# struan-robertson/shoeprint-image-retrieval

Hardware: AMD Instinct MI355X
Metric: query x gallery NCC pairs/sec (higher is better)
Workload: dtype f32; 1 GPU; config 2: WVU2019-shaped VGG16 conv3_3 NCC: Q=100 x G=1500 (1500/GPU), features [256,128,64] stored as float32, rotations/scales none, queries signal 1 / noise 126; method=fft, gallery_chunk=1500, storage=float32, parallelism=gallery-shard x1, streams=1

## Files before the change

### shoeprint-image-retrieval_amd/csrc/ncc_prep6.hip

```cpp
#include "fft_core.h"
#include "ncc_fft_cfg.h"
#include "ncc_prep_common.h"

namespace spr {
namespace {

using C6 = Cfg<12, 16, 12, 8, 384, 5, 2, 1>;
constexpr int kPT = 512;
constexpr int kLoads = 16;
constexpr int kSeg = 4;
constexpr int kRowSeg = 16;
constexpr int kChansPerWg = 8;

#ifdef SPR_PREP6_STAMPS
__device__ unsigned long long g_prep6_stamps[16];
#define SPR_PSTAMP6(i) do { if (blockIdx.x == 12 && blockIdx.y == 700 && c == c_first + 1 && threadIdx.x == 0) g_prep6_stamps[i] = __builtin_amdgcn_s_memtime(); } while (0)
#else
#define SPR_PSTAMP6(i)
#endif

struct Prep6Lds {
  size_t x0_off, f_off, xbuf_off, tw_off, total;
  int f_stride;
};
Prep6Lds prep6_lds(const NccGeom& g) {
  const int h = g.ih, w = g.iw;
  Prep6Lds l;
  l.f_stride = C6::NW / 2 + 1;
  const size_t f_bytes = sizeof(cf) * static_cast<size_t>(2 * ((h + 1) / 2)) * l.f_stride;
  l.x0_off = 64;
  l.f_off = align_up(l.x0_off + sizeof(float) * h * w, 16);
  l.xbuf_off = align_up(l.f_off + f_bytes, 16);
  const size_t fft_total = l.xbuf_off + sizeof(cf) * C6::prep_xbuf_elems(kPT);
  const size_t stat_total = l.f_off + 2 * sizeof(double) * static_cast<size_t>(h) * w;
  l.tw_off = align_up(fft_total > stat_total ? fft_total : stat_total, 16);
  l.total = l.tw_off + sizeof(cf) * (C6::NW + C6::NH);
  return l;
}

__device__ __forceinline__ void stretch_offsets(double t, int sg, int d, double& off, double& tot) {
  const double a = shfl_xor(t, d), b = shfl_xor(t, 2 * d), c = shfl_xor(t, 3 * d);
  off = 0.0;
  tot = 0.0;
#pragma unroll
  for (int j = 0; j < kSeg; ++j) {
    const double v = j == sg ? t : (j == (sg ^ 1) ? a : (j == (sg ^ 2) ? b : c));
    off += j < sg ? v : 0.0;
    tot += v;
  }
}

__global__ void __launch_bounds__(kPT)
prep6_gallery_kernel(NccGeom g, const void* __restrict__ maps, unsigned char* __restrict__ prepared, size_t item_bytes,
                     const cf* __restrict__ tw_h, const cf* __restrict__ tw_w, unsigned x0_off, unsigned f_off,
                     unsigned xbuf_off, unsigned tw_off, int f_stride) {
  using C = C6;
  using GH = typename C::GH;
  using GW = typename C::GW;
  unsigned char* lds = dyn_lds();
  double* red = reinterpret_cast<double*>(lds);
  float* x0 = reinterpret_cast<float*>(lds + x0_off);
  cf* F = reinterpret_cast<cf*>(lds + f_off);
  cf* xbuf = reinterpret_cast<cf*>(lds + xbuf_off);
  const int tid = static_cast<int>(threadIdx.x);
  const size_t item = blockIdx.y;
  const int h = g.ih, w = g.iw, n = h * w;
  double* H1 = reinterpret_cast<double*>(lds + f_off);
  double* H2 = H1 + n;
  const int c_first = static_cast<int>(blockIdx.x) * kChansPerWg;
  const int c_end = c_first + kChansPerWg < g.channels ? c_first + kChansPerWg : g.channels;

  unsigned char* item_base = prepared + item * item_bytes;
  const size_t spec_bytes = sizeof(cf) * static_cast<size_t>(g.channels) * C::kSpecPerChan;
  unsigned char* flags = item_base + spec_bytes + sizeof(float) * static_cast<size_t>(g.channels) * g.inv_per_chan;

  const int dy = kPT / w, dx = kPT - dy * w;
  const int y_first = tid / w, x_first = tid - y_first * w;
  float v[kLoads];
  auto request = [&](int c) {
    const size_t chan_base = (item * g.channels + c) * static_cast<size_t>(g.g_h) * g.g_w;
    int yy = y_first, xx = x_first;
#pragma unroll
    for (int k = 0; k < kLoads; ++k) {
      v[k] = tid + k * kPT < n
                 ? load_feature(maps, chan_base + static_cast<size_t>(yy + g.crop) * g.g_w + (xx + g.crop), g.dtype)
                 : 0.0f;
      xx += dx; yy += dy;
      if (xx >= w) { xx -= w; ++yy; }
    }
  };
  request(c_first);

  cf* twt_w = reinterpret_cast<cf*>(lds + tw_off);
  cf* twt_h = twt_w + C::NW;
  for (int k = tid; k < C::NW; k += kPT) twt_w[k] = tw_w[(k / C::TGW) * (k % C::TGW)];
  for (int k = tid; k < C::NH; k += kPT) twt_h[k] = tw_h[(k / C::TGH) * (k % C::TGH)];

  const int cy = g.th / 2, cx = g.tw / 2;
  const int above = g.th - cy, left = g.tw - cx;
  const double inv_n = 1.0 / (static_cast<double>(g.th) * static_cast<double>(g.tw));

  for (int c = c_first; c < c_end; ++c) {
    SPR_PSTAMP6(0);
    double s = 0.0;
#pragma unroll
    for (int k = 0; k < kLoads; ++k)
      if (tid + k * kPT < n) s += static_cast<double>(v[k]);
    const double total = block_sum(s, red);
    const float mean = static_cast<float>(total / static_cast<double>(n));
    double e = 0.0;
#pragma unroll
    for (int k = 0; k < kLoads; ++k) {
      if (tid + k * kPT < n) {
        const float d = v[k] - mean;
        x0[tid + k * kPT] = d;
        const float sq = d * d;
        e += static_cast<double>(sq);
      }
    }
    SPR_PSTAMP6(1);
    const float energy = static_cast<float>(block_sum(e, red));
    const float rs = energy > 0.0f ? static_cast<float>(1.0 / sqrt(static_cast<double>(energy))) : 0.0f;
    if (tid == 0) flags[c] = rs == 0.0f ? 1 : 0;
    if (c + 1 < c_end) request(c + 1);
    SPR_PSTAMP6(2);

    {
      const int tidv = opaque(tid);
      const int u = tidv < h * kSeg ? tidv : h * kSeg - 1;
      const bool live = tidv < h * kSeg;
      const int y = u / kSeg, sg = u - y * kSeg;
      const int wseg = (w + kSeg - 1) / kSeg;
      const int xa = sg * wseg < w ? sg * wseg : w;
      const int cnt = w - xa < wseg ? w - xa : wseg;
      const float* src = x0 + y * w;
      float tv[kRowSeg];
#pragma unroll
      for (int k = 0; k < kRowSeg; ++k) {
        const float t = src[xa + k < w ? xa + k : w - 1];
        tv[k] = k < cnt ? t : 0.0f;
      }
      double r1 = 0.0, r2 = 0.0;
#pragma unroll
      for (int k = 0; k < kRowSeg; ++k) {
        const float sq = tv[k] * tv[k];
        r1 += static_cast<double>(tv[k]);
        r2 += static_cast<double>(sq);
      }
      double q1, q2, t1, t2;
      stretch_offsets(r1, sg, 1, q1, t1);
      stretch_offsets(r2, sg, 1, q2, t2);
      double* h1 = H1 + y * w;
      double* h2 = H2 + y * w;
      if (live) {
#pragma unroll
        for (int k = 0; k < kRowSeg; ++k) {
          const float sq = tv[k] * tv[k];
          q1 += static_cast<double>(tv[k]);
          q2 += static_cast<double>(sq);
          const int kk = xa + k + 1;
          if (k < cnt && kk < w) {
            const int xl = kk - left;
            if (xl >= 0 && xl <= cx) { h1[xl] = q1; h2[xl] = q2; }
            const int xr = kk + cx;
            if (xr < w) { h1[xr] = t1 - q1; h2[xr] = t2 - q2; }
          }
        }
        if (cnt > 0 && xa + cnt == w) {
          int xl = w - left < 0 ? 0 : w - left;
          const int xe = cx < w - 1 ? cx : w - 1;
          for (; xl <= xe; ++xl) { h1[xl] = q1; h2[xl] = q2; }
        }
      }
    }
    __syncthreads();
    SPR_PSTAMP6(7);

    {
      const int tidv = opaque(tid);
      const int xcol = ((tidv >> 6) & 3) * 16 + (tidv & 15), csg = (tidv >> 4) & 3;
      const int hseg = (h + kSeg - 1) / kSeg;
      const int ya = csg * hseg < h ? csg * hseg : h;
      const int ycnt = xcol < w ? (h - ya < hseg ? h - ya : hseg) : 0;
      double* col = ((tidv >> 8) ? H2 : H1) + ya * w + (xcol < w ? xcol : w - 1);
      constexpr int B = 8;
      double r = 0.0;
      for (int k0 = 0; k0 < ycnt; k0 += B) {
        double t[B];
#pragma unroll
        for (int k = 0; k < B; ++k) t[k] = col[(k0 + k < ycnt ? k0 + k : ycnt - 1) * w];
#pragma unroll
        for (int k = 0; k < B; ++k) r += k0 + k < ycnt ? t[k] : 0.0;
      }
      double run, tot;
      stretch_offsets(r, csg, 16, run, tot);
      for (int k0 = 0; k0 < ycnt; k0 += B) {
        double t[B];
#pragma unroll
        for (int k = 0; k < B; ++k) t[k] = col[(k0 + k < ycnt ? k0 + k : ycnt - 1) * w];
#pragma unroll
        for (int k = 0; k < B; ++k) {
          run += k0 + k < ycnt ? t[k] : 0.0;
          col[(k0 + k < ycnt ? k0 + k : ycnt - 1) * w] = run;
        }
      }
    }
    __syncthreads();
    SPR_PSTAMP6(8);
    {
      float4* inv4 = reinterpret_cast<float4*>(item_base + spec_bytes) + static_cast<size_t>(c) * (g.inv_per_chan / 4);
      for (int idx4 = opaque(tid); idx4 < C::kInv6PerChan / 4; idx4 += kPT) {
        const int pp = idx4 / C::NT, lane6 = idx4 - pp * C::NT;
        const int l64 = lane6 & 63, rg = l64 / 3, tq = l64 - 3 * rg;
        const int row = (lane6 >> 6) * C::kRowGroups + rg, n1 = 3 * pp + tq;
        float o[4] = {0.0f, 0.0f, 0.0f, 0.0f};
        if (l64 < 63 && n1 < 16 && row < h) {
          const int b = (33 * n1) % 48;
          const int ma = tq == 1 ? b - 32 : b, mb = ma == n1 ? n1 + 16 : n1;
          const bool upper = row <= cy;
          const int hi = upper ? (row + above < h ? row + above : h) - 1 : h - 1;
          const int lo = upper ? 0 : row - cy - 1;
          const double* p1a = H1 + hi * w;
          const double* p1b = H1 + lo * w;
          const double* p2a = H2 + hi * w;
          const double* p2b = H2 + lo * w;
          double a1[4], b1[4], a2[4], b2[4];
#pragma unroll
          for (int e = 0; e < 4; ++e) {
            const int x = 2 * (e < 2 ? ma : mb) + (e & 1), xs = x < w ? x : w - 1;
            a1[e] = p1a[xs]; b1[e] = p1b[xs]; a2[e] = p2a[xs]; b2[e] = p2b[xs];
          }
#pragma unroll
          for (int e = 0; e < 4; ++e) {
            const int x = 2 * (e < 2 ? ma : mb) + (e & 1);
            const float r = inv_sigma_from_sums(upper ? a1[e] : a1[e] - b1[e], upper ? a2[e] : a2[e] - b2[e], inv_n);
            o[e] = x < w ? r : 0.0f;
          }
        }
        inv4[idx4] = float4{o[0], o[1], o[2], o[3]};
      }
    }
    __syncthreads();
    SPR_PSTAMP6(3);

    {
      const int tidv = opaque(tid);
      const int giw = tidv / C::TGW, t = tidv - giw * C::TGW;
      const LdsTwiddles<C::TGW> twr{twt_w, t};
      cf* gbuf = xbuf + giw * C::kRowGroupElems;
      cf* zb = gbuf;
      const int pairs = (h + 1) / 2;
      constexpr int kPairsPerRound = kPT / C::TGW;
      const int rounds = ceil_div(pairs, kPairsPerRound);
      for (int rr = 0; rr < rounds; ++rr) {
        const int pr = rr * kPairsPerRound + giw;
        const int ra = 2 * pr, rb = ra + 1;
        cf x[C::EW], y[GW::SPL][C::TGW];
#pragma unroll
        for (int m = 0; m < C::EW; ++m) {
          const int n2 = GW::in_index(t, m);
          const bool in = n2 < w;
          x[m].x = (in && ra < h) ? x0[ra * w + n2] : 0.0f;
          x[m].y = (in && rb < h) ? x0[rb * w + n2] : 0.0f;
        }
        group_fft<C::EW, C::TGW, -1>(x, y, t, twr, gbuf);
        wave_sync();
#pragma unroll
        for (int pp = 0; pp < GW::SPL; ++pp)
#pragma unroll
          for (int sidx = 0; sidx < C::TGW; ++sidx)
            if (GW::out_valid(t, pp)) zb[GW::out_index(t, pp, sidx)] = y[pp][sidx];
        wave_sync();
        if (pr < pairs) {
          for (int k = t; k <= C::NW / 2; k += C::TGW) {
            const cf zk = zb[k];
            const cf zm = zb[k == 0 ? 0 : C::NW - k];
            F[ra * f_stride + k] = cmake(0.5f * (zk.x + zm.x), 0.5f * (zk.y - zm.y));
            F[rb * f_stride + k] = cmake(0.5f * (zk.y + zm.y), 0.5f * (zm.x - zk.x));
          }
        }
        wave_sync();
      }
    }
    __syncthreads();
    SPR_PSTAMP6(4);

    {
      cf* spec = reinterpret_cast<cf*>(item_base) + static_cast<size_t>(c) * C::kSpecPerChan;
      const int tidv = opaque(tid);
      const int gi = tidv / C::TGH, t = tidv - gi * C::TGH;
      const LdsTwiddles<C::TGH> twc{twt_h, t};
      cf* gbuf = xbuf + gi * GH::kGroupElems;
      const int rows_f = 2 * ((h + 1) / 2);
      constexpr int kColsPerRound = kPT / C::TGH;
      constexpr int kRounds = (C::COLS + 1 + kColsPerRound - 1) / kColsPerRound;
      for (int rc = 0; rc < kRounds; ++rc) {
        const int j = rc * kColsPerRound + gi;
        const bool nyq = j == C::COLS;
        const bool active = j <= C::COLS;
        cf x[C::EH], y[GH::SPL][C::TGH];
#pragma unroll
        for (int m = 0; m < C::EH; ++m) {
          const int n1 = GH::in_index(t, m);
          x[m] = (active && n1 < rows_f) ? F[n1 * f_stride + j] : cmake(0.0f, 0.0f);
        }
        group_fft<C::EH, C::TGH, -1>(x, y, t, twc, gbuf);
        if (active) {
#pragma unroll
          for (int pp = 0; pp < GH::SPL; ++pp) {
            if (!GH::out_valid(t, pp)) continue;
#pragma unroll
            for (int sidx = 0; sidx < C::TGH; ++sidx) {
              const int k1 = GH::out_index(t, pp, sidx);
              spec[nyq ? C::kNyqOffset + k1 : C::spec_index(C::slot(j), k1)] = y[pp][sidx];
            }
          }
        }
      }
    }
    __syncthreads();
    SPR_PSTAMP6(5);
  }
}

}

bool prep6_covers(const NccGeom& g) {
  if (!g.six || g.big || !g.prep6) return false;
  if (g.nh != C6::NH || g.nw != C6::NW || g.nt != C6::NT) return false;
  if (g.th < g.ih || g.tw < g.iw) return false;
  if (g.ih > C6::kRows6 || g.ih * kSeg > kPT || g.iw > 64) return false;
  if (g.ih * g.iw > kLoads * kPT) return false;
  if (g.inv_per_chan != C6::kInv6PerChan) return false;
  return prep6_lds(g).total <= static_cast<size_t>(kLdsLimit);
}

int launch_prep6(const NccGeom& g, const PlanScratch& s, const PrepCall& c) {
  const Prep6Lds l = prep6_lds(g);
  const size_t item_bytes = prepared_gallery_item_bytes(g, SPR_NCC_FFT);
  (void)hipFuncSetAttribute(reinterpret_cast<const void*>(prep6_gallery_kernel),
                            hipFuncAttributeMaxDynamicSharedMemorySize, kLdsLimit);
  const size_t elem = g.dtype == SPR_F32 ? 4 : 2;
  const size_t raw_item_bytes = static_cast<size_t>(g.channels) * g.g_h * g.g_w * elem;
  const int64_t batch = 65535;
  for (int64_t first = 0; first < c.n; first += batch) {
    const int64_t m = c.n - first < batch ? c.n - first : batch;
    hipLaunchKernelGGL(prep6_gallery_kernel, dim3(ceil_div(g.channels, kChansPerWg), static_cast<unsigned>(m)), dim3(kPT),
                       l.total, c.stream, g,
                       static_cast<const void*>(static_cast<const unsigned char*>(c.maps) + first * raw_item_bytes),
                       static_cast<unsigned char*>(c.prepared) + first * item_bytes, item_bytes, s.tw_h, s.tw_w,
                       static_cast<unsigned>(l.x0_off), static_cast<unsigned>(l.f_off), static_cast<unsigned>(l.xbuf_off),
                       static_cast<unsigned>(l.tw_off), l.f_stride);
    const int rc = check_launch("prep6_gallery_kernel");
    if (rc != SPR_OK) return rc;
  }
  return SPR_OK;
}

#ifdef SPR_PREP6_STAMPS
extern "C" int spr_debug_read_prep_stamps(unsigned long long* host, int n) {
  return hipMemcpyFromSymbol(host, HIP_SYMBOL(g_prep6_stamps), sizeof(unsigned long long) * n) == hipSuccess ? 0 : -1;
}
#endif

}
```

Baseline: 279,200 pairs/s.

## Remove energy block reduction and prefetch next-channel sum into reduction slots

The per-channel energy block reduction is replaced with two LDS OR-flags that only check whether any squared deviation is positive or overflow-prone. The exact double energy sum now runs only in that rare overflow case. The next channel's sum is reduced per wave during an existing barrier interval, which removes a block_sum from the critical path. The column prefix scan now holds its whole segment in 32 registers instead of loading twice in chunks of 8, and the row-stretch stores are merged into one branch. These changes cut barriers and LDS traffic at the cost of higher register pressure and an extra syncthreads for the flags.

```diff
diff --git a/shoeprint-image-retrieval_amd/csrc/ncc_prep6.hip b/shoeprint-image-retrieval_amd/csrc/ncc_prep6.hip
--- a/shoeprint-image-retrieval_amd/csrc/ncc_prep6.hip
+++ b/shoeprint-image-retrieval_amd/csrc/ncc_prep6.hip
@@ -10,7 +10,10 @@
 constexpr int kLoads = 16;
 constexpr int kSeg = 4;
 constexpr int kRowSeg = 16;
+constexpr int kColSeg = 32;
 constexpr int kChansPerWg = 8;
+static_assert(kColSeg * kSeg >= C6::kRows6, "a column stretch fits its registers");
+constexpr float kSquareBound = 0x1p100f;
 
 #ifdef SPR_PREP6_STAMPS
 __device__ unsigned long long g_prep6_stamps[16];
@@ -28,7 +31,7 @@
   Prep6Lds l;
   l.f_stride = C6::NW / 2 + 1;
   const size_t f_bytes = sizeof(cf) * static_cast<size_t>(2 * ((h + 1) / 2)) * l.f_stride;
-  l.x0_off = 64;
+  l.x0_off = 80;
   l.f_off = align_up(l.x0_off + sizeof(float) * h * w, 16);
   l.xbuf_off = align_up(l.f_off + f_bytes, 16);
   const size_t fft_total = l.xbuf_off + sizeof(cf) * C6::prep_xbuf_elems(kPT);
@@ -59,6 +62,7 @@
   using GW = typename C::GW;
   unsigned char* lds = dyn_lds();
   double* red = reinterpret_cast<double*>(lds);
+  int* orw = reinterpret_cast<int*>(lds + 64);
   float* x0 = reinterpret_cast<float*>(lds + x0_off);
   cf* F = reinterpret_cast<cf*>(lds + f_off);
   cf* xbuf = reinterpret_cast<cf*>(lds + xbuf_off);
@@ -90,11 +94,19 @@
     }
   };
   request(c_first);
+  auto lane_sum = [&]() {
+    double s = 0.0;
+#pragma unroll
+    for (int k = 0; k < kLoads; ++k)
+      if (tid + k * kPT < n) s += static_cast<double>(v[k]);
+    return s;
+  };
 
   cf* twt_w = reinterpret_cast<cf*>(lds + tw_off);
   cf* twt_h = twt_w + C::NW;
   for (int k = tid; k < C::NW; k += kPT) twt_w[k] = tw_w[(k / C::TGW) * (k % C::TGW)];
   for (int k = tid; k < C::NH; k += kPT) twt_h[k] = tw_h[(k / C::TGH) * (k % C::TGH)];
+  if (tid < 2) orw[tid] = 0;
 
   const int cy = g.th / 2, cx = g.tw / 2;
   const int above = g.th - cy, left = g.tw - cx;
@@ -102,26 +114,45 @@
 
   for (int c = c_first; c < c_end; ++c) {
     SPR_PSTAMP6(0);
-    double s = 0.0;
-#pragma unroll
-    for (int k = 0; k < kLoads; ++k)
-      if (tid + k * kPT < n) s += static_cast<double>(v[k]);
-    const double total = block_sum(s, red);
+    double total = 0.0;
+    if (c == c_first) {
+      total = block_sum(lane_sum(), red);
+    } else {
+#pragma unroll
+      for (int wv = 0; wv < kPT / 64; ++wv) total += red[wv];
+    }
     const float mean = static_cast<float>(total / static_cast<double>(n));
-    double e = 0.0;
+    bool pos = false, big = false;
 #pragma unroll
     for (int k = 0; k < kLoads; ++k) {
       if (tid + k * kPT < n) {
         const float d = v[k] - mean;
         x0[tid + k * kPT] = d;
         const float sq = d * d;
-        e += static_cast<double>(sq);
-      }
-    }
+        pos |= sq > 0.0f;
+        big |= !(sq < kSquareBound);
+      }
+    }
+    if (pos) orw[0] = 1;
+    if (big) orw[1] = 1;
     SPR_PSTAMP6(1);
-    const float energy = static_cast<float>(block_sum(e, red));
-    const float rs = energy > 0.0f ? static_cast<float>(1.0 / sqrt(static_cast<double>(energy))) : 0.0f;
-    if (tid == 0) flags[c] = rs == 0.0f ? 1 : 0;
+    __syncthreads();
+    bool dead = orw[0] == 0;
+    if (orw[1] != 0) {
+      double e = 0.0;
+#pragma unroll
+      for (int k = 0; k < kLoads; ++k) {
+        if (tid + k * kPT < n) {
+          const float d = v[k] - mean;
+          const float sq = d * d;
+          e += static_cast<double>(sq);
+        }
+      }
+      const float energy = static_cast<float>(block_sum(e, red));
+      const float rs = energy > 0.0f ? static_cast<float>(1.0 / sqrt(static_cast<double>(energy))) : 0.0f;
+      dead = rs == 0.0f;
+    }
+    if (tid == 0) flags[c] = dead ? 1 : 0;
     if (c + 1 < c_end) request(c + 1);
     SPR_PSTAMP6(2);
 
@@ -159,11 +190,11 @@
           q1 += static_cast<double>(tv[k]);
           q2 += static_cast<double>(sq);
           const int kk = xa + k + 1;
-          if (k < cnt && kk < w) {
-            const int xl = kk - left;
-            if (xl >= 0 && xl <= cx) { h1[xl] = q1; h2[xl] = q2; }
-            const int xr = kk + cx;
-            if (xr < w) { h1[xr] = t1 - q1; h2[xr] = t2 - q2; }
+          const bool pre = kk >= left;
+          const int xp = pre ? kk - left : kk + cx;
+          if (k < cnt && kk < w && xp <= (pre ? cx : w - 1)) {
+            h1[xp] = pre ? q1 : t1 - q1;
+            h2[xp] = pre ? q2 : t2 - q2;
           }
         }
         if (cnt > 0 && xa + cnt == w) {
@@ -174,6 +205,7 @@
       }
     }
     __syncthreads();
+    if (tid < 2) orw[tid] = 0;
     SPR_PSTAMP6(7);
 
     {
@@ -182,26 +214,21 @@
       const int hseg = (h + kSeg - 1) / kSeg;
       const int ya = csg * hseg < h ? csg * hseg : h;
       const int ycnt = xcol < w ? (h - ya < hseg ? h - ya : hseg) : 0;
-      double* col = ((tidv >> 8) ? H2 : H1) + ya * w + (xcol < w ? xcol : w - 1);
-      constexpr int B = 8;
+      double* col = ((tidv >> 8) ? H2 : H1) + (ycnt > 0 ? ya * w + xcol : 0);
+      const int last = ycnt > 0 ? ycnt - 1 : 0;
+      double t[kColSeg];
+#pragma unroll
+      for (int k = 0; k < kColSeg; ++k) t[k] = col[(k < last ? k : last) * w];
       double r = 0.0;
-      for (int k0 = 0; k0 < ycnt; k0 += B) {
-        double t[B];
-#pragma unroll
-        for (int k = 0; k < B; ++k) t[k] = col[(k0 + k < ycnt ? k0 + k : ycnt - 1) * w];
-#pragma unroll
-        for (int k = 0; k < B; ++k) r += k0 + k < ycnt ? t[k] : 0.0;
-      }
+#pragma unroll
+      for (int k = 0; k < kColSeg; ++k) r += k < ycnt ? t[k] : 0.0;
       double run, tot;
       stretch_offsets(r, csg, 16, run, tot);
-      for (int k0 = 0; k0 < ycnt; k0 += B) {
-        double t[B];
-#pragma unroll
-        for (int k = 0; k < B; ++k) t[k] = col[(k0 + k < ycnt ? k0 + k : ycnt - 1) * w];
-#pragma unroll
-        for (int k = 0; k < B; ++k) {
-          run += k0 + k < ycnt ? t[k] : 0.0;
-          col[(k0 + k < ycnt ? k0 + k : ycnt - 1) * w] = run;
+      if (ycnt > 0) {
+#pragma unroll
+        for (int k = 0; k < kColSeg; ++k) {
+          run += k < ycnt ? t[k] : 0.0;
+          col[(k < last ? k : last) * w] = run;
         }
       }
     }
@@ -242,6 +269,13 @@
     }
     __syncthreads();
     SPR_PSTAMP6(3);
+
+    if (c + 1 < c_end) {
+      double s = lane_sum();
+      for (int m = 32; m >= 1; m >>= 1) s += shfl_xor(s, m);
+      if ((tid & 63) == 0) red[tid >> 6] = s;
+    }
+    SPR_PSTAMP6(9);
 
     {
       const int tidv = opaque(tid);
```

New measurement: 281,500 pairs/s, median of 6. About the same (+0.8%).
